# chenjianqu/dynamic_vins

Measured on AMD Instinct MI355X. Metric: stereo frames/sec (track+BA), higher is better.
Workload: dtype f64; 1 GPU; synthetic 1280x720 stereo @20 Hz + IMU @200 Hz, ZED intrinsics with distortion, figure-8 in a textured box room, max_cnt 250, min_dist 25, flow_back 1, 10 solver iterations, BA + marginalization on every frame; mode=raw, config=zed, parallelism=replicas x1 (independent sequences, no collective), landmarks_in_window=266, features_per_frame=250, warmup_requested=5, gpu_max_hw_queues=4, frames=resident in HBM before the timed region

## Files before the change

### dynamic_vins_amd/csrc/be_api.hip

```cpp
#include <algorithm>
#include <atomic>
#include <condition_variable>
#include <mutex>
#include "dv_ctx.h"
#include "be_kernels.h"

static_assert(sizeof(dv_ba_factor) == sizeof(BeFactor), "public/private factor layouts must match");
static_assert(sizeof(dv_ba_lm) == sizeof(BeLm), "public/private landmark layouts must match");
static_assert(sizeof(dv_ba_prior) == sizeof(BePriorHdr), "public/private prior layouts must match");

static int be_ensure(dv_ctx* ctx, int nfac) {
    BeWork& w = ctx->be;
    if (w.ready && nfac <= w.fac_cap) return 0;
    const int fac_cap = std::max(nfac, BE_MAX_LM * BE_MAX_OBS_FACTORS);
    size_t off = 0;
    auto take = [&](size_t bytes) { size_t o = off; off += (bytes + 255) / 256 * 256; return o; };
    const size_t n = BE_MAX_STATE;
    size_t o_ctl = take(sizeof(BeCtl)), o_x = take(sizeof(BeState)), o_imu = take(sizeof(BeImu) * BE_WIN), o_pr = take(sizeof(BePriorHdr)), o_i = take(4 * 4 * n),
           o_mt = take(4 * BE_MARG_TAB_INTS), o_lm = take(sizeof(BeLm) * BE_MAX_LM), o_fac = take(sizeof(BeFactor) * (size_t)fac_cap);
    const size_t upload_bytes = off;
    size_t o_c = take(sizeof(BeState)),
           o_pA = take(8 * (size_t)BE_MAX_PRIOR * BE_MAX_PRIOR), o_pb = take(8 * BE_MAX_PRIOR),
           o_pA2 = take(8 * (size_t)BE_MAX_PRIOR * BE_MAX_PRIOR), o_pb2 = take(8 * BE_MAX_PRIOR), o_ms = take(64), o_c0 = take(64),
           o_pk = take(8 * (size_t)BE_PK_SIZE * BE_PK_STRIDE), o_io = take(8 * (size_t)BE_WIN * IMU_OUT_STRIDE), o_po = take(8 * (BE_MAX_PRIOR + 1)),
// ... 469 lines not shown
    ea.dims = d; ea.g_norm = P->g_norm; ea.cand_cost = w.cand_cost; ea.lm_obs = w.lm_obs; ea.prior_c0 = w.prior_c0 + w.prior_cur;
    ea.lm_lo = 0; ea.lm_hi = P->nlm;
    if (P->free_blocks & 3) {
        if (ctx->dist.transport != 0) DV_FAIL("dv_ba_solve: free extrinsic / td blocks are not built for the landmark-sharded window");
        if (xt.on) {
            DV_CHECK(w.xpk_buf.ensure(2 * 8 * (size_t)BX_SIZE * BE_PK_STRIDE));
            xt.xpk[0] = (double*)w.xpk_buf.p; xt.xpk[1] = xt.xpk[0] + (size_t)BX_SIZE * BE_PK_STRIDE;
        }
    }
    BeShard sh{};
    if (ctx->dist.transport != 0) {
        const DvDist& dd = ctx->dist;
        sh.on = 1; sh.rank = dd.rank; sh.world = dd.world;
        sh.cap = std::max(1, (P->nlm + dd.world - 1) / dd.world);
        sh.lo = std::min(P->nlm, dd.rank * sh.cap); sh.hi = std::min(P->nlm, sh.lo + sh.cap);
        sh.len = BE_XS_LEN;
        sh.xsend = (double*)dd.xsend.p; sh.xrecv = (const double*)dd.xrecv.p;
        sh.qf[0] = (double*)dd.qf.p; sh.qf[1] = sh.qf[0] + BE_QF_LEN;
        ea.lm_lo = sh.lo; ea.lm_hi = sh.hi;
    }
    for (int k = 0; k < 2; ++k) { ea.packets[k] = w.packets[k]; ea.imu_out[k] = w.imu_out[k]; ea.prior_out[k] = w.prior_out[k]; }
    BeSolveArgs sa{};
    sa.ctl = w.ctl; sa.x = w.x; sa.cand = w.cand; sa.lm = w.lm; sa.imu = w.imu; sa.prior = w.prior; sa.priorA = w.priorA; sa.dims = d;
    sa.cand_cost = w.cand_cost; sa.lm_obs = w.lm_obs;
    for (int k = 0; k < 2; ++k) { sa.packets[k] = w.packets[k]; sa.imu_out[k] = w.imu_out[k]; sa.prior_out[k] = w.prior_out[k]; sa.Hd[k] = w.Hd[k]; sa.Sc[k] = w.Sc[k]; sa.gvec[k] = w.gvec[k]; }
    sa.scale_p = w.scale_p; sa.diag_p = w.diag_p; sa.grad_p = w.grad_p; sa.gn_p = w.gn_p; sa.scale_l = w.scale_l; sa.diag_l = w.diag_l; sa.grad_l = w.grad_l; sa.gn_l = w.gn_l;
    sa.prior_col = w.prior_col; sa.col_kind = w.col_kind; sa.col_frame = w.col_frame; sa.col_comp = w.col_comp;
    sa.xnorm2_extra = P->x_norm2_extra; sa.sh = sh; sa.xt = xt;
    sa.ldl_mf16 = 0;
    if (!w.ldl_generic && !(P->free_blocks & 3)) {
        uint8_t plan[64];
        if (be_mf16_plan(d.nstate, plan)) { std::memcpy(sa.ldl_col0, plan, sizeof(plan)); sa.ldl_mf16 = 1; }
    }
    pd.rej_on = false;
    if (fused && fused->want_reject && w.gpu_reject && P->nlm > 0) {
        if (!w.rej_pinned) DV_CHECK(hipHostMalloc((void**)&w.rej_pinned, BE_MAX_LM, hipHostMallocDefault));
        BeRejectArgs& r = pd.rej;
        r.st = w.cand; r.fac = w.fac; r.lm = w.lm; r.nlm = P->nlm; r.nframes = P->nframes; r.focal = fused->rej_focal; r.flags = w.rej_pinned;
        std::memcpy(r.ric, fused->rej_ric, sizeof(r.ric)); std::memcpy(r.tic, fused->rej_tic, sizeof(r.tic));
        r.ex_from_state = (P->free_blocks & 1) ? 1 : 0; r.pad = 0;
        pd.rej_on = true;
    }
    pd.xt = xt; pd.copy_ex_td = (P->free_blocks & 3) != 0;
    pd.ea = ea; pd.sa = sa; pd.fused_present = fused != nullptr; pd.fuse_accept_gauge = fused != nullptr && !ctx->batch && !sh.on ; pd.max_iters = P->max_iters; pd.g_norm = P->g_norm; pd.nframes = P->nframes; pd.use_imu = P->use_imu; pd.nlm = P->nlm;
    pd.want_raw_pose = fused && fused->want_raw_pose;
    if (fused) { std::memcpy(pd.gauge_R0, fused->R0, sizeof(pd.gauge_R0)); std::memcpy(pd.gauge_ypr0, fused->ypr0, sizeof(pd.gauge_ypr0)); std::memcpy(pd.gauge_P0, fused->P0, sizeof(pd.gauge_P0)); }
    pd.do_marg = do_marg; pd.state_bytes = state_bytes; pd.nxt = 1 - w.prior_cur;
    if (eval_only) {
        be_launch_eval(ea, BE_EVAL_X, s); be_launch_eval_ext(ea, xt, BE_EVAL_X, s);
        be_launch_reduce(sa, 0, s); be_launch_reduce_ext(sa, 0, s);
        if (sh.on) { if (be_exchange(ctx, (size_t)sh.len, s)) return -1; be_launch_shard_finalize(sa, 0, s); }
        DV_CHECK(hipGetLastError());
        return 0;
    }
    if (w.debug_hash_log && fused) {
        if (!w.dbg_pinned) DV_CHECK(hipHostMalloc((void**)&w.dbg_pinned, 64, hipHostMallocDefault));
        const size_t up_bytes = w.up_fac + sizeof(BeFactor) * (size_t)P->nfac;
        be_dbg_hash(w.block.p, up_bytes & ~(size_t)7, w.dbg_pinned + 0, s);
        const bool pv = P->prior && P->prior->valid;
        if (pv) { be_dbg_hash(w.priorA, 8 * (size_t)P->prior->n * P->prior->n, w.dbg_pinned + 1, s); be_dbg_hash(w.priorb, 8 * (size_t)P->prior->n, w.dbg_pinned + 2, s); } else { w.dbg_pinned[1] = 0; w.dbg_pinned[2] = 0; }
    }
    const int first_slots = w.debug_short_first_pass ? std::max(1, P->max_iters - 2) : P->max_iters;
    if (ctx->batch && fused && !sh.on) {
        pd.deferred = true; pd.first_slots = first_slots;
        pd.active = true; pd.t_begin = t_begin; pd.t_up = t_up; pd.t_enq = t_up;
        return 0;
// ... 386 lines not shown
    if (last4) std::memcpy(last4, ctx->be.marg_last, 32);
    return 0;
}
int dv_batch_timing(dv_batch* B, int on, double* out3, long long* rounds, int* windows) {
    if (!B) return -1;
    if (on && !B->tev[0]) for (auto& e : B->tev) if (hipEventCreate(&e) != hipSuccess) return -1;
    B->timing = on != 0;
    if (out3) for (int k = 0; k < 3; ++k) out3[k] = B->t_n ? B->t_ms[k] / (double)B->t_n : 0.0;
    if (rounds) *rounds = B->t_n;
    if (windows) *windows = B->t_windows;
    return 0;
}
int dv_batch_info(dv_batch* B, long long* batched_rounds, long long* single_rounds) {
    if (!B) return -1;
    if (batched_rounds) *batched_rounds = B->batched_rounds;
    if (single_rounds) *single_rounds = B->single_rounds;
    return 0;
}

int dv_debug_set(dv_ctx* ctx, const char* key, int value) {
    if (!ctx || !key) return -1;
    if (std::strcmp(key, "short_first_pass") == 0) { ctx->be.debug_short_first_pass = value != 0; return 0; }
    if (std::strcmp(key, "peer_timeout_ms") == 0) { ctx->dist.peer_timeout_ticks = 100000ll * std::max(value, 1); return 0; }
    if (std::strcmp(key, "batch_single_eval") == 0) { ctx->be.debug_batch_single = (ctx->be.debug_batch_single & ~1) | (value ? 1 : 0); return 0; }
    if (std::strcmp(key, "batch_single_reduce") == 0) { ctx->be.debug_batch_single = (ctx->be.debug_batch_single & ~2) | (value ? 2 : 0); return 0; }
    if (std::strcmp(key, "batch_single_tail") == 0) { ctx->be.debug_batch_single = (ctx->be.debug_batch_single & ~8) | (value ? 8 : 0); return 0; }
    if (std::strcmp(key, "batch_single_solve") == 0) { ctx->be.debug_batch_single = (ctx->be.debug_batch_single & ~4) | (value ? 4 : 0); return 0; }
    if (std::strcmp(key, "hash_light") == 0) { ctx->be.debug_hash_light = value != 0; return 0; }
    if (std::strcmp(key, "hash_log") == 0) { ctx->be.debug_hash_log = value != 0; return 0; }
    if (std::strcmp(key, "wait_tail") == 0) { ctx->be.debug_wait_tail = value != 0; return 0; }
    if (std::strcmp(key, "gpu_reject") == 0) { ctx->be.gpu_reject = value != 0; return 0; }
    if (std::strcmp(key, "c0_side") == 0) { ctx->be.c0_side = value != 0; return 0; }
    if (std::strcmp(key, "ldl_generic") == 0) { ctx->be.ldl_generic = value != 0; return 0; }
    DV_FAIL(std::string("dv_debug_set: unknown key ") + key);
}

int dv_ba_eval(dv_ctx* ctx, const dv_ba_problem* P, int* n_out, double* cost, double* S, double* g) {
    if (!ctx) return -1;
    if (!P || !n_out) DV_FAIL("dv_ba_eval: null argument");
    if (ctx->be.pend->active) DV_FAIL("dv_ba_eval: a solve is in flight");
    if (ctx->est && ctx->be.prior_resident && P->prior && P->prior->valid && P->prior_A != ctx->be.priorA_buf[ctx->be.prior_cur])
        DV_FAIL("dv_ba_eval: this ctx's estimator holds a device-resident prior; use a separate ctx for operator-level calls");
    if (be_begin_impl(ctx, const_cast<dv_ba_problem*>(P), nullptr, true)) return -1;
    BeWork& w = ctx->be;
    hipStream_t s = ctx->be_stream;
    const BePending& pd = *w.pend;
    if (pd.trivial) { w.pend->active = false; *n_out = 0; if (cost) *cost = 0; return 0; }
    const int n = pd.sa.dims.nstate, NBR = (n + 3) / 4, nblk = NBR * (NBR + 1) / 2;
    *n_out = n;
    std::vector<double> blk((size_t)nblk * 16), gv(2 * (size_t)n), lcost((size_t)std::max(P->nlm, 1)), io((size_t)std::max(P->nimu, 1) * IMU_OUT_STRIDE), pc(1);
    DV_CHECK(hipMemcpyAsync(blk.data(), w.Sc[0], 8 * blk.size(), hipMemcpyDeviceToHost, s));
    DV_CHECK(hipMemcpyAsync(gv.data(), w.gvec[0], 8 * gv.size(), hipMemcpyDeviceToHost, s));
    if (P->nlm) DV_CHECK(hipMemcpyAsync(lcost.data(), w.packets[0] + (size_t)BE_PK_COST * BE_PK_STRIDE, 8 * (size_t)P->nlm, hipMemcpyDeviceToHost, s));
    if (P->nimu) DV_CHECK(hipMemcpyAsync(io.data(), w.imu_out[0], 8 * (size_t)P->nimu * IMU_OUT_STRIDE, hipMemcpyDeviceToHost, s));
    DV_CHECK(hipMemcpyAsync(pc.data(), w.prior_out[0], 8, hipMemcpyDeviceToHost, s));
    DV_CHECK(hipStreamSynchronize(s));
    if (be_dist_check(ctx)) return -1;
    if (cost) {
        double c = 0;
        if (pd.sa.sh.on) {
            double lc = 0; DV_CHECK(hipMemcpy(&lc, pd.sa.sh.qf[0] + BE_QF_A + 10, 8, hipMemcpyDeviceToHost)); c = lc;
        } else for (int l = 0; l < P->nlm; ++l) c += lcost[l];
        for (int k = 0; k < P->nimu; ++k) c += io[(size_t)k * IMU_OUT_STRIDE];
        c += pc[0]; *cost = c;
    }
    if (g) for (int i = 0; i < n; ++i) g[i] = gv[i] - gv[n + i];
// ... 116 lines not shown
```

### dynamic_vins_amd/csrc/be_kernels.h

```cpp
#pragma once
#include <cstddef>
#include <hip/hip_runtime.h>
#include "be_factor_dev.h"

#define IMU_OUT_STRIDE 936

#define BE_XS_MSZ (66 * 36)
#define BE_XS_M(k) ((k) * BE_XS_MSZ)
#define BE_XS_V(k) (5 * BE_XS_MSZ + (k) * 66)
#define BE_XS_A (5 * BE_XS_MSZ + 8 * 66)
#define BE_XS_LEN (BE_XS_A + 16)
#define BE_XS_BUF ((BE_XS_LEN > BE_MAX_LM + 16 ? BE_XS_LEN : BE_MAX_LM + 16))
#define BE_QF_M(k) ((k) * 4356)
#define BE_QF_V(k) (4 * 4356 + (k) * 66)
#define BE_QF_A (4 * 4356 + 7 * 66)
#define BE_QF_LEN (BE_QF_A + 16)
struct BeShard { int32_t on, rank, world, lo, hi, cap, len, pad; double* xsend; const double* xrecv; double* qf[2]; };

#define BE_NX 13
#define BX_W 0
#define BX_G 13
#define BX_XX 26
#define BX_XP 195
#define BX_SIZE 1056
struct BeExt { int32_t on, pad; int32_t xcol[BE_NX + 1]; double* xpk[2]; };

struct BeEvalArgs {
    const BeCtl* ctl;
    const BeState* x; const BeState* cand;
    const BeFactor* fac; const BeLm* lm; const BeImu* imu; const BePriorHdr* prior; const double* priorA; const double* priorb;
    BeDims dims; double g_norm;
    double* packets[2];
    double* imu_out[2];
    double* prior_out[2];
    double* cand_cost;
    int32_t* lm_obs;
    int32_t lm_lo, lm_hi;
    const double* prior_c0;
};

struct BeSolveArgs {
    BeCtl* ctl;
    BeState* x; BeState* cand;
    const BeLm* lm; const BeImu* imu; const BePriorHdr* prior; const double* priorA;
    BeDims dims;
    const double* packets[2]; const double* imu_out[2]; const double* prior_out[2]; const double* cand_cost; const int32_t* lm_obs;
    double* Hd[2];
    double* Sc[2];
    double* gvec[2];
    double* scale_p; double* diag_p; double* grad_p; double* gn_p;
    double* scale_l; double* diag_l; double* grad_l; double* gn_l;
    int32_t* prior_col;
    int32_t* col_kind; int32_t* col_frame; int32_t* col_comp;
    uint8_t ldl_col0[64]; int32_t ldl_mf16, ldl_pad;
    BeShard sh;
    double xnorm2_extra;
    BeExt xt;
};

struct BeMargArgs {
    const BeState* x; int nframes, nlm, nimu;
    const BeFactor* fac; const BeLm* lm; const BeImu* imu;
    const BePriorHdr* prior; const double* priorA; const double* priorb;
    const int32_t* prior_map;
    const int32_t* imu_map;
    const int32_t* dim_slot;
    const int32_t* dim_comp;
    int D, m; double g_norm;
    double* outA; double* outb; double* out_scalars;
    double* W; double* part; double* psum;
    int pose_dim[BE_NF], ex_dim[2], td_dim;
    int c0_mode;
    double* sum; double* lm_h; int anchor;
    double* imu_w;
    double* c0_out;
    const int32_t* lm_sel;
    uint8_t mf_plan[64]; int32_t mf16, mf_n;
};

struct BeGaugeArgs {
    const BeState* x; BeState* out; int nframes, use_imu, nlm; double R0[9]; double ypr0[3]; double P0[3];
    BeState* h_out; BeCtl* h_ctl; const BeCtl* ctl; double* h_raw_pose; int state_doubles, pad;
};

struct BeRejectArgs { const BeState* st; const BeFactor* fac; const BeLm* lm; int nlm, nframes; double ric[2][9], tic[2][3], focal; uint8_t* flags; int ex_from_state, pad; };
void be_launch_reject(const BeRejectArgs& a, hipStream_t s);

// ... 127 lines not shown
```

### dynamic_vins_amd/csrc/be_solve.hip

```cpp
#include <hip/hip_runtime.h>
#include <cfloat>
#include <algorithm>
#include <cstring>
#include <cstdlib>
#include "be_kernels.h"
#include "dev_once.h"
#include "wave_dpp.h"
#include "be_mf16.h"

using namespace be;

#ifdef BE_RED_TS
__device__ long long be_red_ts[64];
#define RTS(k) do { if (threadIdx.x == 0) be_red_ts[k] = wall_clock64(); } while (0)
extern "C" int dv_debug_red_ts(long long* out) { return hipMemcpyFromSymbol(out, HIP_SYMBOL(be_red_ts), sizeof(long long) * 64) == hipSuccess ? 0 : -1; }
#else
#define RTS(k) do {} while (0)
#endif
#define RED_THREADS 448
#define RED_PAIRS (BE_NF * (BE_NF + 1) / 2)
__device__ const unsigned char RED_PAIR_TAB[RED_PAIRS] = {
    150, 152, 51, 132, 98, 166, 170, 112, 147, 85, 68, 65, 32, 168, 49, 167, 118, 153, 66, 129, 96, 130, 165, 144, 33, 148, 67, 48, 102, 162, 161, 0, 97,
    133, 50, 16, 101, 134, 17, 119, 99, 84, 114, 64, 80, 100, 163, 160, 145, 149, 115, 131, 82, 164, 81, 151, 113, 117, 116, 128, 34, 136, 83, 169, 146, 135 };
__device__ __forceinline__ void red_pair(int bx, int& fi, int& fj) { const int t = RED_PAIR_TAB[bx]; fi = t >> 4; fj = t & 15; }
// ... 650 lines not shown
    const int NBR = (n + 3) >> 2, bi = i >> 2, bj = j >> 2;
    const bool in = i < n;
    return Sc[in ? (size_t)(bj * NBR - bj * (bj - 1) / 2 + bi - bj) * 16 + (i & 3) * 4 + (j & 3) : 0];
}
__device__ __forceinline__ double mf_finish(double raw, const double* v_s, const double* v_d, const double* rhs, int n, double mu, int i, int j) {
    const int hi = i > j ? i : j, lo = i > j ? j : i, hc = hi < n ? hi : n - 1, lc = lo < n ? lo : n - 1;
    const double s_hi = v_s[hc], s_lo = v_s[lc], d_hi = v_d[hc];
    const double body = s_hi * s_lo * raw + (i == j ? mu * d_hi * d_hi : 0.0);
    const double row_n = lo == n ? MF_RHO : s_lo * rhs[lc];
    return hi < n ? body : (hi == n ? row_n : (hi == lo ? 1.0 : 0.0));
}
__device__ __forceinline__ void mf_prefetch(const double* __restrict__ Sc, const uint8_t* plan, int n, mf_d4 (&U)[5]) {
    const int lane = threadIdx.x & 63, wave = mf_wave(), c = lane & 15, rho = lane >> 4;
    int sI[5], sJ[5];
    mf_slots(plan, wave, (n + 16) >> 4, sI, sJ);
    const int NBR = (n + 3) >> 2;
#pragma unroll
    for (int s = 0; s < 5; ++s) {
        if (sI[s] > sJ[s]) {
            const int i = min(16 * sI[s] + c, n - 1);
            const int lane_off = ((i >> 2) << 4) + ((i & 3) << 2) + rho;
#pragma unroll
            for (int r = 0; r < 4; ++r) {
                const int bj = 4 * sJ[s] + r;
                const int bjc = bj < NBR ? bj : 0;
                U[s][r] = Sc[(size_t)((bjc * NBR - bjc * (bjc - 1) / 2 - bjc) << 4) + lane_off];
            }
        } else {
#pragma unroll
            for (int r = 0; r < 4; ++r) U[s][r] = sI[s] >= 0 ? mf_raw(Sc, n, 16 * sI[s] + c, 16 * sJ[s] + rho + 4 * r) : 0.0;
        }
    }
}
template <class Side, class Side0>
__device__ __forceinline__ bool ldlt_mf16(mf_d4 (&U)[MF_SLOTS], const uint8_t* plan, int n, double mu, const double* v_s, const double* v_d, const double* rhs, const MfLds& m, int* s_fail, Side side, Side0 side0) {
    const int tid = threadIdx.x, lane = tid & 63, wave = mf_wave(), c = lane & 15, rho = lane >> 4;
    const int NB = (n + 16) >> 4, IB = n >> 4, c0 = n & 15;
    int sI[MF_SLOTS], sJ[MF_SLOTS];
    mf_slots(plan, wave, NB, sI, sJ);
    TS(21);
#pragma unroll
    for (int s = 0; s < MF_SLOTS; ++s) {
        if (sI[s] > sJ[s]) {
            const int i = 16 * sI[s] + c;
            const double si = v_s[min(i, n - 1)];
#pragma unroll
            for (int r = 0; r < 4; ++r) {
                const int j = 16 * sJ[s] + rho + 4 * r;
                const double sj = v_s[j];
                const double body = si * sj * U[s][r];
                U[s][r] = i < n ? body : (i == n ? sj * rhs[j] : 0.0);
            }
        } else {
#pragma unroll
            for (int r = 0; r < 4; ++r) U[s][r] = sI[s] >= 0 ? mf_finish(U[s][r], v_s, v_d, rhs, n, mu, 16 * sI[s] + c, 16 * sJ[s] + rho + 4 * r) : 0.0;
        }
    }
    TS(22);
    for (int i = tid; i < 16 * NB; i += SOL_THREADS) m.yv[i] = 0.0;
    if (tid == 0) *s_fail = 0;
#ifdef BE_SOLVE_TS
    if (tid == 0) { be_dbg_ts[19] = 0; be_dbg_ts[20] = 0; be_dbg_ts[32] = 0; be_dbg_ts[33] = 0; be_dbg_ts[34] = 0; be_dbg_ts[35] = 0; }
#endif
    lds_barrier();
    TS(4);
    const int k_side = -1;
    if (wave == 0) { mf_diag(U[0], m, 0, NB, n, s_fail); if (k_side < 0) side0(); }
    else if (k_side < 0) side(0);
    lds_barrier();
#ifdef BE_SOLVE_TS
    long long t_prev = wall_clock64(), acc_panel = 0, acc_update = 0;
    if (tid == 0) be_dbg_ts[16] = t_prev - be_dbg_ts[4];
#endif
    auto panel = [&](mf_d4& T, int I, int k) -> mf_d4 {
        const mf_d4 wf = *reinterpret_cast<const mf_d4*>(m.gat + 768 + lane * 4);
        double ivr[4];
#pragma unroll
        for (int q = 0; q < 4; ++q) ivr[q] = m.iv[16 * k + rho + 4 * q];
        mf_d4 Y = { 0.0, 0.0, 0.0, 0.0 };
#pragma unroll
        for (int q = 0; q < 4; ++q) Y = mf_mfma(wf[q], T[q], Y);
        const mf_d4 Y0 = Y;
#pragma unroll
        for (int r = 0; r < 4; ++r) Y[r] *= ivr[r];
        T = Y;
        *reinterpret_cast<mf_d4*>(m.Tl + (size_t)mf_tix(I, k, NB) * 256 + lane * 4) = Y;
        if (I == IB && c == c0) {
#pragma unroll
            for (int r = 0; r < 4; ++r) m.yv[16 * k + rho + 4 * r] = Y[r];
        }
        return Y0;
    };
    for (int k = 0; k + 1 < NB; ++k) {
        if (wave == k + 1) {
            __builtin_amdgcn_s_setprio(3);
#ifdef BE_SOLVE_TS
            const long long t_c0 = wall_clock64();
#endif
            const mf_d4 Y0 = panel(U[1], k + 1, k);
#ifdef BE_SOLVE_TS
            __builtin_amdgcn_s_waitcnt(0xc07f); const long long t_c1 = wall_clock64();
#endif
#pragma unroll
            for (int q = 0; q < 4; ++q) U[0] = mf_mfma(U[1][q], -Y0[q], U[0]);
#ifdef BE_SOLVE_TS
            asm volatile("s_nop 15\n\ts_nop 3\n\tv_mov_b64 %0, %0" : "+v"(U[0][0])); const long long t_c2 = wall_clock64();
#endif
            if (k + 2 < NB) lds_barrier();
#ifdef BE_SOLVE_TS
            const long long t_u = wall_clock64();
            if (lane == 0) { be_dbg_ts[32] += t_c0 - t_prev; be_dbg_ts[33] += t_c1 - t_c0; be_dbg_ts[34] += t_c2 - t_c1; be_dbg_ts[35] += t_u - t_c2; }
#endif
            mf_diag(U[0], m, k + 1, NB, n, s_fail);
#ifdef BE_SOLVE_TS
            if (lane == 0) { be_dbg_ts[19] += wall_clock64() - t_u; be_dbg_ts[20] += t_u - t_prev; }
#endif
            lds_barrier();
        } else {
#pragma unroll
            for (int s = 1; s < MF_SLOTS; ++s) if (sJ[s] == k) panel(U[s], sI[s], k);
            if (k + 2 < NB) lds_barrier();
#ifdef BE_SOLVE_TS
            { const long long t = wall_clock64(); acc_panel += t - t_prev; t_prev = t; }
#endif
            double dk[4];
#pragma unroll
            for (int q = 0; q < 4; ++q) dk[q] = -m.dv[16 * k + rho + 4 * q];
#pragma unroll
            for (int s = 0; s < MF_SLOTS; ++s) if (sJ[s] > k) {
                const mf_d4 a = *reinterpret_cast<const mf_d4*>(m.Tl + (size_t)mf_tix(sJ[s], k, NB) * 256 + lane * 4);
                const mf_d4 b = *reinterpret_cast<const mf_d4*>(m.Tl + (size_t)mf_tix(sI[s], k, NB) * 256 + lane * 4);
#pragma unroll
                for (int q = 0; q < 4; ++q) U[s] = mf_mfma(a[q], dk[q] * b[q], U[s]);
            }
            if (k == k_side) side(k + 1);
            if (k == k_side + 1 && k_side >= 0 && wave == k_side + 1) side0();
            lds_barrier();
#ifdef BE_SOLVE_TS
            { const long long t = wall_clock64(); acc_update += t - t_prev; t_prev = t; }
#endif
        }
    }
    if (tid < n) { const double d = m.dv[tid]; if (!(d > 0.0) || !isfinite(d)) *s_fail = 1; }
    lds_barrier();
    TS(5);
#ifdef BE_SOLVE_TS
    if (tid == 0) { be_dbg_ts[17] = acc_panel; be_dbg_ts[18] = acc_update; }
#endif
    return *s_fail == 0;
}
#ifndef MF_BS_PERMLANE
#define MF_BS_PERMLANE 1
#endif
typedef unsigned mf_u2 __attribute__((ext_vector_type(2)));
__device__ __forceinline__ double mf_rows4_sum(double v) {
    mf_u2 a = __builtin_amdgcn_permlane32_swap((unsigned)__double2loint(v), (unsigned)__double2loint(v), false, false);
    mf_u2 b = __builtin_amdgcn_permlane32_swap((unsigned)__double2hiint(v), (unsigned)__double2hiint(v), false, false);
    const double t = __hiloint2double((int)b[0], (int)a[0]) + __hiloint2double((int)b[1], (int)a[1]);
    a = __builtin_amdgcn_permlane16_swap((unsigned)__double2loint(t), (unsigned)__double2loint(t), false, false);
    b = __builtin_amdgcn_permlane16_swap((unsigned)__double2hiint(t), (unsigned)__double2hiint(t), false, false);
    return __hiloint2double((int)b[0], (int)a[0]) + __hiloint2double((int)b[1], (int)a[1]);
}
__device__ __forceinline__ void bs_mf16(const uint8_t* plan, int n, const MfLds& m, double* v_x) {
    const int tid = threadIdx.x, lane = tid & 63, wave = mf_wave(), c = lane & 15, rho = lane >> 4;
    const int NB = (n + 16) >> 4, IB = n >> 4, c0 = n & 15;
    int sI[MF_SLOTS], sJ[MF_SLOTS];
    mf_slots(plan, wave, NB, sI, sJ);
    double* gat = m.gat + wave * 64;
    for (int i = NB - 1; i >= 0; --i) {
        bool need = wave == 0;
#pragma unroll
        for (int s = 1; s < MF_SLOTS; ++s) need = need || sI[s] == i;
        if (need) {
            const mf_d4 Wi = *reinterpret_cast<const mf_d4*>(m.Tl + (size_t)mf_tix(i, i, NB) * 256 + lane * 4);
            double part = 0.0;
#pragma unroll
            for (int r = 0; r < 4; ++r) part = __builtin_fma(Wi[r], m.yv[16 * i + rho + 4 * r], part);
            double xi = MF_BS_PERMLANE ? mf_rows4_sum(part) : 0.0;
            if (!MF_BS_PERMLANE) {
                gat[lane] = part;
                wave_lds_sync();
                xi = (gat[c] + gat[16 + c]) + (gat[32 + c] + gat[48 + c]);
                wave_lds_sync();
            }
            if (i == IB && c >= c0) xi = 0.0;
            if (wave == 0 && rho == 0 && 16 * i + c < n) v_x[16 * i + c] = xi;
#pragma unroll
            for (int s = 1; s < MF_SLOTS; ++s) if (sI[s] == i) {
                const double* V = m.Tl + (size_t)mf_tix(i, sJ[s], NB) * 256;
                gat[lane] = xi;
                wave_lds_sync();
                double acc = 0.0;
#pragma unroll
                for (int q = 0; q < 4; ++q) { const int C = rho + 4 * q; acc = __builtin_fma(V[((((c & 3) << 4) + C) << 2) + (c >> 2)], gat[C], acc); }
                wave_lds_sync();
                double t = MF_BS_PERMLANE ? mf_rows4_sum(acc) : 0.0;
                if (!MF_BS_PERMLANE) {
                    gat[lane] = acc;
                    wave_lds_sync();
                    t = (gat[c] + gat[16 + c]) + (gat[32 + c] + gat[48 + c]);
                    wave_lds_sync();
                }
                if (rho == 0) m.yv[16 * sJ[s] + c] -= t;
            }
        }
        lds_barrier();
    }
}

template <int SEG, int ROWS>
__device__ __forceinline__ void bs_chunk(const double* Lm, int kt, int lane, double& x0, double& x1, double& x2) {
    double cr[ROWS][3];
#pragma unroll
    for (int u = 0; u < ROWS; ++u) {
        const int k = kt - u;
        const double* row = Lm + tri(k, 0) + lane;
        cr[u][0] = row[0];
        if (SEG >= 1) cr[u][1] = row[64];
        if (SEG >= 2) cr[u][2] = row[128];
        cr[u][SEG] = lane < k - 64 * SEG ? cr[u][SEG] : 0.0;
    }
#pragma unroll
    for (int u = 0; u < ROWS; ++u) {
        const int k = kt - u;
        const double xs = SEG == 0 ? x0 : (SEG == 1 ? x1 : x2);
        const int lo = __builtin_amdgcn_readlane(__double2loint(xs), k - 64 * SEG), hi = __builtin_amdgcn_readlane(__double2hiint(xs), k - 64 * SEG);
        const double xk = __hiloint2double(hi, lo);
        x0 = __builtin_fma(-cr[u][0], xk, x0);
        if (SEG >= 1) x1 = __builtin_fma(-cr[u][1], xk, x1);
        if (SEG >= 2) x2 = __builtin_fma(-cr[u][2], xk, x2);
    }
}
template <int SEG, int R>
__device__ __forceinline__ void bs_ld(const double* Lm, int kt, int lane, double (&cr)[R][3]) {
#pragma unroll
    for (int u = 0; u < R; ++u) {
        const int k = kt - u;
        const double* row = Lm + tri(k, 0) + lane;
        cr[u][0] = row[0];
        if (SEG >= 1) cr[u][1] = row[64];
// ... 124 lines not shown
```

### dynamic_vins_amd/csrc/be_solve_body.inc

```
    extern __shared__ __attribute__((aligned(16))) double sm[];
    BeCtl* ctl = a.ctl;
    BeCtl c = *ctl;
    const int n = a.dims.nstate, nlm = a.dims.nlm, tid = threadIdx.x;
    const int lm0 = SHARD ? a.sh.lo : 0, nown = SHARD ? a.sh.hi - a.sh.lo : nlm;
    if (c.done) return;
    __shared__ int s_pcol[BE_NF], s_scol[BE_NF];
    if (tid < BE_NF) { s_pcol[tid] = tid < a.dims.nframes ? a.dims.pose_col[tid] : -1; s_scol[tid] = tid < a.dims.nframes ? a.dims.sb_col[tid] : -1; }
    __shared__ int s_xcol[MF16 ? 1 : 16]; __shared__ double qx[MF16 ? 1 : 16];
    bool xt_on = false;
    if constexpr (!MF16) { xt_on = a.xt.on != 0; if (tid >= 64 && tid < 80) s_xcol[tid - 64] = (xt_on && tid - 64 < BE_NX) ? a.xt.xcol[tid - 64] : -1; }
    TS(15);
    const int cur_spec = (spec && c.pending) ? (c.cur ^ 1) : c.cur;
    double dec_cv[4] = { 0.0, 0.0, 0.0, 0.0 };
    if (MF16 && spec && c.pending && tid < 256) {
        const int ncost0 = nlm + a.dims.nimu + 1;
#pragma unroll
        for (int u = 0; u < 4; ++u) dec_cv[u] = a.cand_cost[tid + 256 * u < ncost0 ? tid + 256 * u : 0];
    }
    mf_d4 mfU[MF_SLOTS];
    double pre_h = 0.0, pre_g0 = 0.0, pre_g1 = 0.0, pre_s = 0.0;
    if (MF16 && !(c.reuse && !(spec && c.pending))) {
        mf_prefetch(a.Sc[cur_spec], reinterpret_cast<const uint8_t*>(a.ldl_col0), n, mfU);
        if (tid < n) { pre_h = a.Hd[cur_spec][(size_t)tid * n + tid]; pre_g0 = a.gvec[cur_spec][tid]; pre_g1 = a.gvec[cur_spec][n + tid]; pre_s = a.scale_p[tid]; }
    }
// ... 168 lines not shown
                if (SHARD && tid == 0) part += qfc[BE_QF_A + 10];
                const double xc = block_sum(part, red);
                if (tid == 0) { ctl->x_cost = xc; ctl->initial_cost = xc; }
            }
            {
                double gm = 0;
                for (int i = tid; i < n; i += SOL_THREADS) gm = fmax(gm, fabs(gvec[i]));
                if (!SHARD) for (int l = tid; l < nlm; l += SOL_THREADS) gm = fmax(gm, fabs(BE_PK(pk, BE_PK_G, l)));
                else if (tid == 0) gm = fmax(gm, qfc[BE_QF_A + 11]);
    #pragma unroll
                for (int o = 32; o > 0; o >>= 1) gm = fmax(gm, __shfl_xor(gm, o));
                __syncthreads();
                if ((tid & 63) == 0) red[tid >> 6] = gm;
                __syncthreads();
                gm = 0; for (int k = 0; k < SOL_THREADS / 64; ++k) gm = fmax(gm, red[k]);
                __syncthreads();
                if (gm <= 1e-10) { if (tid == 0) { ctl->done = 1; ctl->termination = 1; ctl->first = 0; } return true; }
            }
            TS(1);
            if (lm_live) {
                const int l = lmi;
                const double h = BE_PK(pk, BE_PK_H, l), gl = BE_PK(pk, BE_PK_G, l), s = a.scale_l[l];
                double d2 = h * s * s; d2 = fmin(fmax(d2, 1e-6), 1e32);
                const double d = sqrt(d2);
                a.diag_l[l] = d; a.grad_l[l] = gl * s / d;
                lm_h = h; lm_g = gl; lm_scale = s; lm_diag = d; lm_grad = gl * s / d;
            }
            return false;
        };
        if (!MF16) { if (cost_and_tolerance()) return; }
        TS(3);
        bool ok_f;
        if (MF16) ok_f = ldlt_mf16(mfU, reinterpret_cast<const uint8_t*>(a.ldl_col0), n, mu, v_s, v_d, v_x, mf, &s_fail, [&](int excl) { side_sums(tid < 64 * excl ? tid : tid - 64, SOL_THREADS - 64, false); },
                                   [&]() { lm_diag_own(); if ((tid & 63) == 0) { red[tid >> 6] = 0.0; red[16 + (tid >> 6)] = 0.0; } });
        else ok_f = ldlt_blocked<NSLOT>(a.Sc[c.cur], gvec, n, mu, v_s, v_d, Lm, PL, PD, dinfo, zfin, dvec, &s_fail);
        if (!ok_f) {
            if (MF16) { if (cost_and_tolerance()) return; }
            if (tid == 0) {
                ctl->mu = mu * 10.0; ctl->chol_fail = 1; ctl->first = 0; ctl->alpha_valid = 0;
                ctl->slots = c.slots + 1; ctl->reuse = 0; ctl->need_eval = 0; ctl->pending = 0;
                if (mu * 10.0 > 1.0) { ctl->done = 1; ctl->termination = 2; }
            }
            return;
        }
        TS(6);
        if (MF16) bs_mf16(reinterpret_cast<const uint8_t*>(a.ldl_col0), n, mf, v_x);
        else if ((tid >> 6) == 0) {
            __builtin_amdgcn_s_setprio(3);
            const int lane = tid & 63, nn = n;
            double x0 = lane < nn ? zfin[lane] / dvec[lane] : 0.0;
            double x1 = 64 + lane < nn ? zfin[64 + lane] / dvec[64 + lane] : 0.0;
            double x2 = 128 + lane < nn ? zfin[128 + lane] / dvec[128 + lane] : 0.0;
            int k = nn - 1;
            for (; k >= 0 && ((k + 1) & 7); --k) bs_rows<1>(Lm, k, lane, x0, x1, x2);
            if (k >= 128 + BS_R - 1) k = bs_segment<2, BS_R>(Lm, k, lane, x0, x1, x2);
            if (k >= 64 + BS_R - 1) k = bs_segment<1, BS_R>(Lm, k, lane, x0, x1, x2);
            if (k >= BS_R - 1) k = bs_segment<0, BS_R>(Lm, k, lane, x0, x1, x2);
            __builtin_amdgcn_s_setprio(0);
            if (lane < nn) v_x[lane] = x0;
            if (64 + lane < nn) v_x[64 + lane] = x1;
            if (128 + lane < nn) v_x[128 + lane] = x2;
        }
        lds_barrier();
        if (MF16) {
            double gm = 0, xc = 0;
            for (int k = 0; k < SOL_THREADS / 64; ++k) { gm = fmax(gm, red[k]); xc += red[16 + k]; }
            if (c.first && tid == 0) { ctl->x_cost = xc; ctl->initial_cost = xc; }
            if (gm <= 1e-10) { if (tid == 0) { ctl->done = 1; ctl->termination = 1; ctl->first = 0; } return; }
        }
        TS(24);
        if (MF16) for (int i = tid; i < n; i += SOL_THREADS) { if (c.first) a.scale_p[i] = v_s[i]; a.diag_p[i] = v_d[i]; a.grad_p[i] = v_grad[i]; }
        TS(7);
        for (int i = tid; i < n; i += SOL_THREADS) { v_gn[i] = -v_d[i] * v_x[i]; a.gn_p[i] = v_gn[i]; v_t[i] = v_s[i] * v_x[i]; }
        lds_barrier();
        gather66(v_t);
        wdot_all();
        if (lm_live) {
            const double rho = 1.0 / (lm_h + mu * lm_diag * lm_diag / (lm_scale * lm_scale));
            lm_wgn = wd[tid];
// ... 221 lines not shown
```

### dynamic_vins_amd/csrc/dv_ctx.h

```cpp
#pragma once
#include "dv_internal.h"
#include "be_types.h"
#include "be_kernels.h"
#include <cmath>
#include <cstring>
#include <chrono>
#include <deque>
#include <map>
#include <memory>
#include <mutex>
#include <string>
#include <vector>

struct DevBuf {
    void* p = nullptr; size_t bytes = 0;
    hipError_t ensure(size_t n) {
        if (n <= bytes) return hipSuccess;
        if (p) (void)hipFree(p);
        p = nullptr; bytes = 0;
        hipError_t e = hipMalloc(&p, n);
        if (e == hipSuccess) bytes = n;
        return e;
    }
    void release() { if (p) (void)hipFree(p); p = nullptr; bytes = 0; }
// ... 54 lines not shown
    bool fuse_accept_gauge = false;
    bool active = false, trivial = false, do_marg = false, fused_present = false, marg_in_flight = false, marg_check_due = false; int scal_slot = 0, check_slot = 0; size_t state_bytes = 0; int nxt = 0; MargPlan pl;
    BeExt xt{}; bool copy_ex_td = false;
    BeEvalArgs ea; BeSolveArgs sa; int max_iters = 0, nframes = 0, use_imu = 0, nlm = 0; double g_norm = 0, gauge_R0[9], gauge_ypr0[3], gauge_P0[3];
    std::chrono::steady_clock::time_point t_begin, t_up, t_enq;
};

struct BeWork {
    std::unique_ptr<BePending> pend = std::make_unique<BePending>();
    bool ready = false;
    DevBuf block;
    BeCtl* ctl = nullptr; BeState* x = nullptr; BeState* cand = nullptr;
    BeFactor* fac = nullptr; BeLm* lm = nullptr; BeImu* imu = nullptr; BePriorHdr* prior = nullptr; double* priorA = nullptr; double* priorb = nullptr;
    double* packets[2] = { nullptr, nullptr }; double* imu_out[2] = { nullptr, nullptr }; double* prior_out[2] = { nullptr, nullptr }; double* cand_cost = nullptr; int32_t* lm_obs = nullptr;
    double* Hd[2] = { nullptr, nullptr }; double* Sc[2] = { nullptr, nullptr }; double* gvec[2] = { nullptr, nullptr };
    double* scale_p = nullptr; double* diag_p = nullptr; double* grad_p = nullptr; double* gn_p = nullptr;
    double* scale_l = nullptr; double* diag_l = nullptr; double* grad_l = nullptr; double* gn_l = nullptr;
    int32_t* prior_col = nullptr; int32_t* col_kind = nullptr; int32_t* col_frame = nullptr; int32_t* col_comp = nullptr;
    int fac_cap = 0;
    DevBuf marg_buf;
    DevBuf xpk_buf;
    void* pinned = nullptr; size_t pinned_bytes = 0;
    size_t up_ctl = 0, up_x = 0, up_imu = 0, up_prior = 0, up_idx = 0, up_mt = 0, up_lm = 0, up_fac = 0, dl_off = 0;
    double* priorA_buf[2] = { nullptr, nullptr }; double* priorb_buf[2] = { nullptr, nullptr }; int prior_cur = 0;
    bool prior_resident = false;
    hipEvent_t ev_state = nullptr;
    hipStream_t c0_stream = nullptr; hipEvent_t ev_margA = nullptr, ev_c0 = nullptr; bool c0_side = false, c0_pending = false;
    double* prior_c0 = nullptr;
    int marg_form = 0;
    DevBuf eig_spec; bool eig_ran = false;
    int32_t* marg_tab = nullptr; double* marg_scal = nullptr;
    long long marg_checked = 0; double marg_last[4] = { 0, 0, 0, 0 };
    long long marg_clamped = 0;
    bool debug_short_first_pass = false, ldl_generic = false, debug_wait_tail = false; int debug_batch_single = 0; bool debug_hash_log = false, debug_hash_light = false;
    std::vector<unsigned long long> dbg_dev_log; unsigned long long* dbg_pinned = nullptr; unsigned long long dbg_solve_no = 0;
    static constexpr int DBG_RANGES = 16, DBG_SLOTS = 16;
    unsigned long long* dbg_slots = nullptr; std::vector<unsigned long long> dbg_slot_log;
    bool gpu_reject = true; uint8_t* rej_pinned = nullptr;
    std::vector<const double*> sqrt_hint;
};

bool be_imu_sqrt_info(const double* cov15x15, double* U15x15);

struct BeFused {
    int marg_mode = -1;
    double R0[9], ypr0[3], P0[3];
    dv_ba_prior new_prior;
    double diag[4] = { 0, 0, 0, 0 };
    bool want_raw_pose = false;
    bool want_reject = false; double rej_ric[2][9], rej_tic[2][3], rej_focal = 0; const uint8_t* rej_flags = nullptr;
    double raw_pose[77];
};
int be_solve_fused(dv_ctx* ctx, dv_ba_problem* P, dv_ba_summary* summary, BeFused* fused);
void be_batch_detach(dv_ctx* ctx);
struct DvFrontBatch;
DvFrontBatch*& be_batch_front(struct dv_batch* B);
int be_batch_index(struct dv_batch* B);
const std::vector<dv_ctx*>& be_batch_members(struct dv_batch* B);
void dv_front_batch_release(DvFrontBatch* F);
void dv_front_batch_sync(DvFrontBatch* F);
void* be_staging_factors(dv_ctx* ctx, int* cap);
int be_solve_fused_begin(dv_ctx* ctx, dv_ba_problem* P, BeFused* fused);
int be_solve_fused_end(dv_ctx* ctx, dv_ba_problem* P, dv_ba_summary* summary, BeFused* fused);
struct dv_obj_problem;
struct ObjPending {
    bool active = false; void* pinned = nullptr; size_t pinned_bytes = 0, up_bytes = 0; hipEvent_t ev = nullptr; hipStream_t stream = nullptr; int V = 0, nblk = 0, n_obj = 0;
    void release() { if (pinned) (void)hipHostFree(pinned); pinned = nullptr; pinned_bytes = 0; if (ev) (void)hipEventDestroy(ev); ev = nullptr; active = false; }
// ... 95 lines not shown
```

Measured before the change: 1201 frames/s.

## Replace serial MF16 back-substitution with inverse-based parallel solve built during factorization

During the MFMA-tiled LDLT factorization, idle waves now build block rows of the inverse of L (Z tiles) and partial solution terms, stored into the lower-triangle tile storage. The back-substitution then becomes a parallel per-wave matrix-vector product over those Z tiles instead of a serial block chain. The new path is the default, and the old chained back-substitution stays available through a debug key. The aim is to cut the latency-bound serial back-solve inside each solver iteration, at the cost of extra MFMA work and LDS traffic inside the factorization loop, plus some numerical-ordering differences.

```diff
diff --git a/dynamic_vins_amd/csrc/be_api.hip b/dynamic_vins_amd/csrc/be_api.hip
--- a/dynamic_vins_amd/csrc/be_api.hip
+++ b/dynamic_vins_amd/csrc/be_api.hip
@@ -525,6 +525,7 @@
         uint8_t plan[64];
         if (be_mf16_plan(d.nstate, plan)) { std::memcpy(sa.ldl_col0, plan, sizeof(plan)); sa.ldl_mf16 = 1; }
     }
+    sa.bs_chain = w.bs_chain ? 1 : 0;
     pd.rej_on = false;
     if (fused && fused->want_reject && w.gpu_reject && P->nlm > 0) {
         if (!w.rej_pinned) DV_CHECK(hipHostMalloc((void**)&w.rej_pinned, BE_MAX_LM, hipHostMallocDefault));
@@ -977,6 +978,7 @@
     if (std::strcmp(key, "gpu_reject") == 0) { ctx->be.gpu_reject = value != 0; return 0; }
     if (std::strcmp(key, "c0_side") == 0) { ctx->be.c0_side = value != 0; return 0; }
     if (std::strcmp(key, "ldl_generic") == 0) { ctx->be.ldl_generic = value != 0; return 0; }
+    if (std::strcmp(key, "bs_chain") == 0) { ctx->be.bs_chain = value != 0; return 0; }
     DV_FAIL(std::string("dv_debug_set: unknown key ") + key);
 }
 
diff --git a/dynamic_vins_amd/csrc/be_kernels.h b/dynamic_vins_amd/csrc/be_kernels.h
--- a/dynamic_vins_amd/csrc/be_kernels.h
+++ b/dynamic_vins_amd/csrc/be_kernels.h
@@ -52,7 +52,7 @@
     double* scale_l; double* diag_l; double* grad_l; double* gn_l;
     int32_t* prior_col;
     int32_t* col_kind; int32_t* col_frame; int32_t* col_comp;
-    uint8_t ldl_col0[64]; int32_t ldl_mf16, ldl_pad;
+    uint8_t ldl_col0[64]; int32_t ldl_mf16, bs_chain;
     BeShard sh;
     double xnorm2_extra;
     BeExt xt;
diff --git a/dynamic_vins_amd/csrc/be_solve.hip b/dynamic_vins_amd/csrc/be_solve.hip
--- a/dynamic_vins_amd/csrc/be_solve.hip
+++ b/dynamic_vins_amd/csrc/be_solve.hip
@@ -706,123 +706,6 @@
         }
     }
 }
-template <class Side, class Side0>
-__device__ __forceinline__ bool ldlt_mf16(mf_d4 (&U)[MF_SLOTS], const uint8_t* plan, int n, double mu, const double* v_s, const double* v_d, const double* rhs, const MfLds& m, int* s_fail, Side side, Side0 side0) {
-    const int tid = threadIdx.x, lane = tid & 63, wave = mf_wave(), c = lane & 15, rho = lane >> 4;
-    const int NB = (n + 16) >> 4, IB = n >> 4, c0 = n & 15;
-    int sI[MF_SLOTS], sJ[MF_SLOTS];
-    mf_slots(plan, wave, NB, sI, sJ);
-    TS(21);
-#pragma unroll
-    for (int s = 0; s < MF_SLOTS; ++s) {
-        if (sI[s] > sJ[s]) {
-            const int i = 16 * sI[s] + c;
-            const double si = v_s[min(i, n - 1)];
-#pragma unroll
-            for (int r = 0; r < 4; ++r) {
-                const int j = 16 * sJ[s] + rho + 4 * r;
-                const double sj = v_s[j];
-                const double body = si * sj * U[s][r];
-                U[s][r] = i < n ? body : (i == n ? sj * rhs[j] : 0.0);
-            }
-        } else {
-#pragma unroll
-            for (int r = 0; r < 4; ++r) U[s][r] = sI[s] >= 0 ? mf_finish(U[s][r], v_s, v_d, rhs, n, mu, 16 * sI[s] + c, 16 * sJ[s] + rho + 4 * r) : 0.0;
-        }
-    }
-    TS(22);
-    for (int i = tid; i < 16 * NB; i += SOL_THREADS) m.yv[i] = 0.0;
-    if (tid == 0) *s_fail = 0;
-#ifdef BE_SOLVE_TS
-    if (tid == 0) { be_dbg_ts[19] = 0; be_dbg_ts[20] = 0; be_dbg_ts[32] = 0; be_dbg_ts[33] = 0; be_dbg_ts[34] = 0; be_dbg_ts[35] = 0; }
-#endif
-    lds_barrier();
-    TS(4);
-    const int k_side = -1;
-    if (wave == 0) { mf_diag(U[0], m, 0, NB, n, s_fail); if (k_side < 0) side0(); }
-    else if (k_side < 0) side(0);
-    lds_barrier();
-#ifdef BE_SOLVE_TS
-    long long t_prev = wall_clock64(), acc_panel = 0, acc_update = 0;
-    if (tid == 0) be_dbg_ts[16] = t_prev - be_dbg_ts[4];
-#endif
-    auto panel = [&](mf_d4& T, int I, int k) -> mf_d4 {
-        const mf_d4 wf = *reinterpret_cast<const mf_d4*>(m.gat + 768 + lane * 4);
-        double ivr[4];
-#pragma unroll
-        for (int q = 0; q < 4; ++q) ivr[q] = m.iv[16 * k + rho + 4 * q];
-        mf_d4 Y = { 0.0, 0.0, 0.0, 0.0 };
-#pragma unroll
-        for (int q = 0; q < 4; ++q) Y = mf_mfma(wf[q], T[q], Y);
-        const mf_d4 Y0 = Y;
-#pragma unroll
-        for (int r = 0; r < 4; ++r) Y[r] *= ivr[r];
-        T = Y;
-        *reinterpret_cast<mf_d4*>(m.Tl + (size_t)mf_tix(I, k, NB) * 256 + lane * 4) = Y;
-        if (I == IB && c == c0) {
-#pragma unroll
-            for (int r = 0; r < 4; ++r) m.yv[16 * k + rho + 4 * r] = Y[r];
-        }
-        return Y0;
-    };
-    for (int k = 0; k + 1 < NB; ++k) {
-        if (wave == k + 1) {
-            __builtin_amdgcn_s_setprio(3);
-#ifdef BE_SOLVE_TS
-            const long long t_c0 = wall_clock64();
-#endif
-            const mf_d4 Y0 = panel(U[1], k + 1, k);
-#ifdef BE_SOLVE_TS
-            __builtin_amdgcn_s_waitcnt(0xc07f); const long long t_c1 = wall_clock64();
-#endif
-#pragma unroll
-            for (int q = 0; q < 4; ++q) U[0] = mf_mfma(U[1][q], -Y0[q], U[0]);
-#ifdef BE_SOLVE_TS
-            asm volatile("s_nop 15\n\ts_nop 3\n\tv_mov_b64 %0, %0" : "+v"(U[0][0])); const long long t_c2 = wall_clock64();
-#endif
-            if (k + 2 < NB) lds_barrier();
-#ifdef BE_SOLVE_TS
-            const long long t_u = wall_clock64();
-            if (lane == 0) { be_dbg_ts[32] += t_c0 - t_prev; be_dbg_ts[33] += t_c1 - t_c0; be_dbg_ts[34] += t_c2 - t_c1; be_dbg_ts[35] += t_u - t_c2; }
-#endif
-            mf_diag(U[0], m, k + 1, NB, n, s_fail);
-#ifdef BE_SOLVE_TS
-            if (lane == 0) { be_dbg_ts[19] += wall_clock64() - t_u; be_dbg_ts[20] += t_u - t_prev; }
-#endif
-            lds_barrier();
-        } else {
-#pragma unroll
-            for (int s = 1; s < MF_SLOTS; ++s) if (sJ[s] == k) panel(U[s], sI[s], k);
-            if (k + 2 < NB) lds_barrier();
-#ifdef BE_SOLVE_TS
-            { const long long t = wall_clock64(); acc_panel += t - t_prev; t_prev = t; }
-#endif
-            double dk[4];
-#pragma unroll
-            for (int q = 0; q < 4; ++q) dk[q] = -m.dv[16 * k + rho + 4 * q];
-#pragma unroll
-            for (int s = 0; s < MF_SLOTS; ++s) if (sJ[s] > k) {
-                const mf_d4 a = *reinterpret_cast<const mf_d4*>(m.Tl + (size_t)mf_tix(sJ[s], k, NB) * 256 + lane * 4);
-                const mf_d4 b = *reinterpret_cast<const mf_d4*>(m.Tl + (size_t)mf_tix(sI[s], k, NB) * 256 + lane * 4);
-#pragma unroll
-                for (int q = 0; q < 4; ++q) U[s] = mf_mfma(a[q], dk[q] * b[q], U[s]);
-            }
-            if (k == k_side) side(k + 1);
-            if (k == k_side + 1 && k_side >= 0 && wave == k_side + 1) side0();
-            lds_barrier();
-#ifdef BE_SOLVE_TS
-            { const long long t = wall_clock64(); acc_update += t - t_prev; t_prev = t; }
-#endif
-        }
-    }
-    if (tid < n) { const double d = m.dv[tid]; if (!(d > 0.0) || !isfinite(d)) *s_fail = 1; }
-    lds_barrier();
-    TS(5);
-#ifdef BE_SOLVE_TS
-    if (tid == 0) { be_dbg_ts[17] = acc_panel; be_dbg_ts[18] = acc_update; }
-#endif
-    return *s_fail == 0;
-}
 #ifndef MF_BS_PERMLANE
 #define MF_BS_PERMLANE 1
 #endif
@@ -834,6 +717,198 @@
     a = __builtin_amdgcn_permlane16_swap((unsigned)__double2loint(t), (unsigned)__double2loint(t), false, false);
     b = __builtin_amdgcn_permlane16_swap((unsigned)__double2hiint(t), (unsigned)__double2hiint(t), false, false);
     return __hiloint2double((int)b[0], (int)a[0]) + __hiloint2double((int)b[1], (int)a[1]);
+}
+__device__ __forceinline__ int zinv_mates(int x, int s) { return s == 0 ? x >> 2 : (x >= s ? ((x - s) >> 2) + 1 : 0); }
+__device__ __forceinline__ const mf_d4& mf_tile(const MfLds& m, int I, int J, int NB) { return *reinterpret_cast<const mf_d4*>(m.Tl + (size_t)mf_tix(I, J, NB) * 256 + (threadIdx.x & 63) * 4); }
+__device__ __forceinline__ double mf_tile_t(const MfLds& m, int I, int J, int NB, int C, int c) { return m.Tl[(size_t)mf_tix(I, J, NB) * 256 + ((((c & 3) << 4) + C) << 2) + (c >> 2)]; }
+__device__ __forceinline__ mf_d4 zinv_row(const MfLds& m, int NB, int k, int wave, int& zj, double* zx) {
+    const int s = (k + 1) & 3;
+    const int lane = threadIdx.x & 63, c = lane & 15, rho = lane >> 4;
+    mf_d4 Z = { 0.0, 0.0, 0.0, 0.0 };
+    if (wave < 1 || wave > k) return Z;
+    const int nm = zinv_mates(wave - 1, s);
+    const int j = (wave & 3) != s ? wave - 1 - nm : k - zinv_mates(k, s) + nm;
+    mf_d4 S = { 0.0, 0.0, 0.0, 0.0 }, zt;
+    for (int mm = j; mm < k; ++mm) {
+        const mf_d4 lt = mf_tile(m, k, mm, NB);
+        zt = mf_tile(m, mm, j, NB);
+#pragma unroll
+        for (int q = 0; q < 4; ++q) S = mf_mfma(lt[q], zt[q], S);
+    }
+#pragma unroll
+    for (int q = 0; q < 4; ++q) Z = mf_mfma(-mf_tile_t(m, k, k, NB, rho + 4 * q, c), S[q], Z);
+    double part = 0.0;
+#pragma unroll
+    for (int r = 0; r < 4; ++r) part = __builtin_fma(zt[r], m.yv[16 * (k - 1) + rho + 4 * r], part);
+    const double xs = mf_rows4_sum(part);
+    if (rho == 0) zx[16 * j + c] = (j == k - 1 ? 0.0 : zx[16 * j + c]) + xs;
+    zj = j;
+    return Z;
+}
+__device__ __forceinline__ void zinv_tail_rows(const MfLds& m, int n, int wave, double* zx, double* zw) {
+    const int NB = (n + 16) >> 4, IB = n >> 4, c0 = n & 15;
+    const int lane = threadIdx.x & 63, c = lane & 15, rho = lane >> 4;
+    if (wave > (IB >= 2 ? IB - 2 : 0)) return;
+    double* gat = m.gat + wave * 64;
+    const mf_d4 Wl = mf_tile(m, IB, IB, NB);
+    double part = 0.0;
+#pragma unroll
+    for (int r = 0; r < 4; ++r) part = __builtin_fma(Wl[r], m.yv[16 * IB + rho + 4 * r], part);
+    double u = mf_rows4_sum(part);
+    if (c >= c0) u = 0.0;
+    if (wave == 0 && rho == 0 && c < c0) zx[16 * IB + c] = u;
+    if (IB == 0) return;
+    gat[lane] = u;
+    wave_lds_sync();
+    double acc = 0.0;
+#pragma unroll
+    for (int q = 0; q < 4; ++q) acc = __builtin_fma(mf_tile_t(m, IB, IB - 1, NB, rho + 4 * q, c), gat[rho + 4 * q], acc);
+    wave_lds_sync();
+    const double yh = m.yv[16 * (IB - 1) + c] - mf_rows4_sum(acc);
+    gat[lane] = yh;
+    wave_lds_sync();
+    const mf_d4 W1 = mf_tile(m, IB - 1, IB - 1, NB);
+    part = 0.0;
+#pragma unroll
+    for (int r = 0; r < 4; ++r) part = __builtin_fma(W1[r], gat[rho + 4 * r], part);
+    wave_lds_sync();
+    const double t = mf_rows4_sum(part);
+    if (wave == 0 && rho == 0) zx[16 * (IB - 1) + c] = t;
+    if (IB < 2) return;
+    gat[lane] = rho == 0 ? u : t;
+    wave_lds_sync();
+    acc = 0.0;
+#pragma unroll
+    for (int q = 0; q < 4; ++q) {
+        acc = __builtin_fma(mf_tile_t(m, IB, wave, NB, rho + 4 * q, c), gat[rho + 4 * q], acc);
+        acc = __builtin_fma(mf_tile_t(m, IB - 1, wave, NB, rho + 4 * q, c), gat[16 + rho + 4 * q], acc);
+    }
+    const double v = mf_rows4_sum(acc);
+    if (rho == 0) zw[16 * wave + c] = (wave == IB - 2 ? m.yv[16 * wave + c] : 0.0) - v;
+}
+template <class Side, class Side0>
+__device__ __forceinline__ bool ldlt_mf16(mf_d4 (&U)[MF_SLOTS], const uint8_t* plan, int n, double mu, const double* v_s, const double* v_d, const double* rhs, const MfLds& m, int* s_fail, Side side, Side0 side0,
+                                          bool zinv, double* zx, double* zw) {
+    const int tid = threadIdx.x, lane = tid & 63, wave = mf_wave(), c = lane & 15, rho = lane >> 4;
+    const int NB = (n + 16) >> 4, IB = n >> 4, c0 = n & 15;
+    int sI[MF_SLOTS], sJ[MF_SLOTS];
+    mf_slots(plan, wave, NB, sI, sJ);
+    TS(21);
+#pragma unroll
+    for (int s = 0; s < MF_SLOTS; ++s) {
+        if (sI[s] > sJ[s]) {
+            const int i = 16 * sI[s] + c;
+            const double si = v_s[min(i, n - 1)];
+#pragma unroll
+            for (int r = 0; r < 4; ++r) {
+                const int j = 16 * sJ[s] + rho + 4 * r;
+                const double sj = v_s[j];
+                const double body = si * sj * U[s][r];
+                U[s][r] = i < n ? body : (i == n ? sj * rhs[j] : 0.0);
+            }
+        } else {
+#pragma unroll
+            for (int r = 0; r < 4; ++r) U[s][r] = sI[s] >= 0 ? mf_finish(U[s][r], v_s, v_d, rhs, n, mu, 16 * sI[s] + c, 16 * sJ[s] + rho + 4 * r) : 0.0;
+        }
+    }
+    TS(22);
+    for (int i = tid; i < 16 * NB; i += SOL_THREADS) m.yv[i] = 0.0;
+    if (tid == 0) *s_fail = 0;
+#ifdef BE_SOLVE_TS
+    if (tid == 0) { be_dbg_ts[19] = 0; be_dbg_ts[20] = 0; be_dbg_ts[32] = 0; be_dbg_ts[33] = 0; be_dbg_ts[34] = 0; be_dbg_ts[35] = 0; }
+#endif
+    lds_barrier();
+    TS(4);
+    const int k_side = -1;
+    if (wave == 0) { mf_diag(U[0], m, 0, NB, n, s_fail); if (k_side < 0) side0(); }
+    else if (k_side < 0) side(0);
+    lds_barrier();
+#ifdef BE_SOLVE_TS
+    long long t_prev = wall_clock64(), acc_panel = 0, acc_update = 0;
+    if (tid == 0) be_dbg_ts[16] = t_prev - be_dbg_ts[4];
+#endif
+    auto panel = [&](mf_d4& T, int I, int k) -> mf_d4 {
+        const mf_d4 wf = *reinterpret_cast<const mf_d4*>(m.gat + 768 + lane * 4);
+        double ivr[4];
+#pragma unroll
+        for (int q = 0; q < 4; ++q) ivr[q] = m.iv[16 * k + rho + 4 * q];
+        mf_d4 Y = { 0.0, 0.0, 0.0, 0.0 };
+#pragma unroll
+        for (int q = 0; q < 4; ++q) Y = mf_mfma(wf[q], T[q], Y);
+        const mf_d4 Y0 = Y;
+#pragma unroll
+        for (int r = 0; r < 4; ++r) Y[r] *= ivr[r];
+        T = Y;
+        *reinterpret_cast<mf_d4*>(m.Tl + (size_t)mf_tix(I, k, NB) * 256 + lane * 4) = Y;
+        if (I == IB && c == c0) {
+#pragma unroll
+            for (int r = 0; r < 4; ++r) m.yv[16 * k + rho + 4 * r] = Y[r];
+        }
+        return Y0;
+    };
+    for (int k = 0; k + 1 < NB; ++k) {
+        if (wave == k + 1) {
+            __builtin_amdgcn_s_setprio(3);
+#ifdef BE_SOLVE_TS
+            const long long t_c0 = wall_clock64();
+#endif
+            const mf_d4 Y0 = panel(U[1], k + 1, k);
+#ifdef BE_SOLVE_TS
+            __builtin_amdgcn_s_waitcnt(0xc07f); const long long t_c1 = wall_clock64();
+#endif
+#pragma unroll
+            for (int q = 0; q < 4; ++q) U[0] = mf_mfma(U[1][q], -Y0[q], U[0]);
+#ifdef BE_SOLVE_TS
+            asm volatile("s_nop 15\n\ts_nop 3\n\tv_mov_b64 %0, %0" : "+v"(U[0][0])); const long long t_c2 = wall_clock64();
+#endif
+            if (k + 2 < NB) lds_barrier();
+#ifdef BE_SOLVE_TS
+            const long long t_u = wall_clock64();
+            if (lane == 0) { be_dbg_ts[32] += t_c0 - t_prev; be_dbg_ts[33] += t_c1 - t_c0; be_dbg_ts[34] += t_c2 - t_c1; be_dbg_ts[35] += t_u - t_c2; }
+#endif
+            mf_diag(U[0], m, k + 1, NB, n, s_fail);
+#ifdef BE_SOLVE_TS
+            if (lane == 0) { be_dbg_ts[19] += wall_clock64() - t_u; be_dbg_ts[20] += t_u - t_prev; }
+#endif
+            lds_barrier();
+        } else {
+#pragma unroll
+            for (int s = 1; s < MF_SLOTS; ++s) if (sJ[s] == k) panel(U[s], sI[s], k);
+            if (k + 2 < NB) lds_barrier();
+#ifdef BE_SOLVE_TS
+            { const long long t = wall_clock64(); acc_panel += t - t_prev; t_prev = t; }
+#endif
+            double dk[4];
+#pragma unroll
+            for (int q = 0; q < 4; ++q) dk[q] = -m.dv[16 * k + rho + 4 * q];
+#pragma unroll
+            for (int s = 0; s < MF_SLOTS; ++s) if (sJ[s] > k) {
+                const mf_d4 a = *reinterpret_cast<const mf_d4*>(m.Tl + (size_t)mf_tix(sJ[s], k, NB) * 256 + lane * 4);
+                const mf_d4 b = *reinterpret_cast<const mf_d4*>(m.Tl + (size_t)mf_tix(sI[s], k, NB) * 256 + lane * 4);
+#pragma unroll
+                for (int q = 0; q < 4; ++q) U[s] = mf_mfma(a[q], dk[q] * b[q], U[s]);
+            }
+            if (k == k_side) side(k + 1);
+            if (k == k_side + 1 && k_side >= 0 && wave == k_side + 1) side0();
+            int zj = -1;
+            mf_d4 zs;
+            if (zinv && k >= 1 && k + 2 <= IB) zs = zinv_row(m, NB, k, wave, zj, zx);
+            lds_barrier();
+            if (zj >= 0) *reinterpret_cast<mf_d4*>(m.Tl + (size_t)mf_tix(k, zj, NB) * 256 + lane * 4) = zs;
+#ifdef BE_SOLVE_TS
+            { const long long t = wall_clock64(); acc_update += t - t_prev; t_prev = t; }
+#endif
+        }
+    }
+    TS(37);
+    if (tid < n) { const double d = m.dv[tid]; if (!(d > 0.0) || !isfinite(d)) *s_fail = 1; }
+    if (zinv) zinv_tail_rows(m, n, wave, zx, zw);
+    lds_barrier();
+    TS(5);
+#ifdef BE_SOLVE_TS
+    if (tid == 0) { be_dbg_ts[17] = acc_panel; be_dbg_ts[18] = acc_update; }
+#endif
+    return *s_fail == 0;
 }
 __device__ __forceinline__ void bs_mf16(const uint8_t* plan, int n, const MfLds& m, double* v_x) {
     const int tid = threadIdx.x, lane = tid & 63, wave = mf_wave(), c = lane & 15, rho = lane >> 4;
@@ -880,6 +955,20 @@
         }
         lds_barrier();
     }
+}
+
+__device__ __forceinline__ void bs_zinv(int n, const MfLds& m, const double* zw, double* zx) {
+    const int lane = threadIdx.x & 63, wave = mf_wave(), c = lane & 15, rho = lane >> 4;
+    const int NB = (n + 16) >> 4, IB = n >> 4, j = wave;
+    if (j > IB - 2) return;
+    double acc = 0.0;
+    for (int mm = j; mm <= IB - 2; ++mm) {
+        const mf_d4 zt = mf_tile(m, mm, j, NB);
+#pragma unroll
+        for (int r = 0; r < 4; ++r) acc = __builtin_fma(zt[r], zw[16 * mm + rho + 4 * r], acc);
+    }
+    const double xs = mf_rows4_sum(acc);
+    if (rho == 0) zx[16 * j + c] = (j == IB - 2 ? 0.0 : zx[16 * j + c]) + xs;
 }
 
 template <int SEG, int ROWS>
diff --git a/dynamic_vins_amd/csrc/be_solve_body.inc b/dynamic_vins_amd/csrc/be_solve_body.inc
--- a/dynamic_vins_amd/csrc/be_solve_body.inc
+++ b/dynamic_vins_amd/csrc/be_solve_body.inc
@@ -224,7 +224,7 @@
         TS(3);
         bool ok_f;
         if (MF16) ok_f = ldlt_mf16(mfU, reinterpret_cast<const uint8_t*>(a.ldl_col0), n, mu, v_s, v_d, v_x, mf, &s_fail, [&](int excl) { side_sums(tid < 64 * excl ? tid : tid - 64, SOL_THREADS - 64, false); },
-                                   [&]() { lm_diag_own(); if ((tid & 63) == 0) { red[tid >> 6] = 0.0; red[16 + (tid >> 6)] = 0.0; } });
+                                   [&]() { lm_diag_own(); if ((tid & 63) == 0) { red[tid >> 6] = 0.0; red[16 + (tid >> 6)] = 0.0; } }, a.bs_chain == 0, v_x, v_t);
         else ok_f = ldlt_blocked<NSLOT>(a.Sc[c.cur], gvec, n, mu, v_s, v_d, Lm, PL, PD, dinfo, zfin, dvec, &s_fail);
         if (!ok_f) {
             if (MF16) { if (cost_and_tolerance()) return; }
@@ -236,7 +236,7 @@
             return;
         }
         TS(6);
-        if (MF16) bs_mf16(reinterpret_cast<const uint8_t*>(a.ldl_col0), n, mf, v_x);
+        if (MF16) { if (a.bs_chain) bs_mf16(reinterpret_cast<const uint8_t*>(a.ldl_col0), n, mf, v_x); else bs_zinv(n, mf, v_t, v_x); }
         else if ((tid >> 6) == 0) {
             __builtin_amdgcn_s_setprio(3);
             const int lane = tid & 63, nn = n;
diff --git a/dynamic_vins_amd/csrc/dv_ctx.h b/dynamic_vins_amd/csrc/dv_ctx.h
--- a/dynamic_vins_amd/csrc/dv_ctx.h
+++ b/dynamic_vins_amd/csrc/dv_ctx.h
@@ -110,7 +110,7 @@
     int32_t* marg_tab = nullptr; double* marg_scal = nullptr;
     long long marg_checked = 0; double marg_last[4] = { 0, 0, 0, 0 };
     long long marg_clamped = 0;
-    bool debug_short_first_pass = false, ldl_generic = false, debug_wait_tail = false; int debug_batch_single = 0; bool debug_hash_log = false, debug_hash_light = false;
+    bool debug_short_first_pass = false, ldl_generic = false, bs_chain = false, debug_wait_tail = false; int debug_batch_single = 0; bool debug_hash_log = false, debug_hash_light = false;
     std::vector<unsigned long long> dbg_dev_log; unsigned long long* dbg_pinned = nullptr; unsigned long long dbg_solve_no = 0;
     static constexpr int DBG_RANGES = 16, DBG_SLOTS = 16;
     unsigned long long* dbg_slots = nullptr; std::vector<unsigned long long> dbg_slot_log;
```

Result: faster. 1221 frames/s (median of 6 runs) (+1.7%).
